# returaj/gan_mpc

Hardware: AMD Instinct MI355X
Metric: trajectories/sec (rollout+backward+critic step) at batch=1024, H=50 (higher is better)
Workload: dtype f32

## Files before the change

### gan_mpc_amd/csrc/gmpc_linearize_sparse.hip

```cpp
#include <cstdio>
#include <type_traits>

#include "gmpc_launch.h"

typedef float f32x4 __attribute__((ext_vector_type(4)));
typedef unsigned v4u __attribute__((ext_vector_type(4)));
typedef unsigned v2u __attribute__((ext_vector_type(2)));

#define GMPC_LIN_PADROWS 24
#define GMPC_SP_H 200
#define GMPC_SP_Z 200
#define GMPC_SP_STR 220
#define GMPC_SP_CAP 216
#define GMPC_SP_WAVE_BYTES (16 * GMPC_SP_STR * 4 + 3 * GMPC_SP_CAP * 4)
#define GMPC_SP_RD 3
#define GMPC_SP_ROW 256

static bool sparse_form(int L, const int* dims, int n, int m) {
  const int Lh = L - 1;
  if (Lh < 2 || n + m > 32 || n < 1) return false;
  for (int l = 1; l <= Lh; ++l)
    if (dims[l] != GMPC_SP_H) return false;
  return true;
}

__global__ void k_pack_sparse(const float* W, float* dst) {
  const int e = blockIdx.x * blockDim.x + threadIdx.x;
  if (e >= GMPC_SP_H * GMPC_SP_H) return;
  const int i = e / GMPC_SP_H, o = e - i * GMPC_SP_H;
  const int t = i >> 4;
  const int slot = i < 192 ? 64 * (t >> 2) + 4 * (i & 15) + (t & 3) : i;
  dst[(size_t)o * GMPC_SP_ROW + slot] = W[e];
}

size_t gmpc_linsparse_floats(int L, const int* dims, int n, int m) {
  if (!sparse_form(L, dims, n, m)) return 0;
  return (size_t)(L - 2) * (GMPC_SP_H + GMPC_LIN_PADROWS) * GMPC_SP_ROW + GMPC_SP_ROW;
}

void gmpc_linsparse_prepare(const MlpDesc& dyn, int n, int m, float* p, LinPad* out, hipStream_t s) {
  for (int l = 0; l < GMPC_MAX_LAYERS; ++l) out->WSP[l] = nullptr;
  if (!sparse_form(dyn.L, dyn.dims, n, m)) return;
  p = reinterpret_cast<float*>((reinterpret_cast<uintptr_t>(p) + 1023) & ~(uintptr_t)1023);
  for (int l = 1; l < dyn.L - 1; ++l) {
    out->WSP[l] = p;
    hipLaunchKernelGGL(k_pack_sparse, dim3((GMPC_SP_H * GMPC_SP_H + 255) / 256), dim3(256), 0, s, dyn.W[l], p);
    p += (size_t)(GMPC_SP_H + GMPC_LIN_PADROWS) * GMPC_SP_ROW;
  }
}

__global__ __launch_bounds__(GMPC_THREADS, 2) void k_linearize_sparse(
    int NSamp, int T, int n, int m, int Lh, LinPad lp, const uint32_t* masks, const int* active, float* AB,
    int samp_mul, int samp_add) {
  extern __shared__ __attribute__((aligned(16))) char smem[];
  const int lane = threadIdx.x & 63, wave = __builtin_amdgcn_readfirstlane(threadIdx.x >> 6);
  const int g = lane >> 4, l16 = lane & 15;
  const int nm = n + m;
  const int nrow = n < 16 ? n : 16;
  char* wbase = smem + wave * GMPC_SP_WAVE_BYTES;
  float* st = reinterpret_cast<float*>(wbase);
  unsigned* lk = reinterpret_cast<unsigned*>(wbase + 16 * GMPC_SP_STR * 4);
  unsigned* lt = lk + GMPC_SP_CAP;
  if (lane < 16 * 8) st[(lane >> 3) * GMPC_SP_STR + GMPC_SP_H + (lane & 7)] = 0.f;
  if (lane + 64 < 16 * 8) st[((lane + 64) >> 3) * GMPC_SP_STR + GMPC_SP_H + (lane & 7)] = 0.f;

  const int lw = l16 * 16, lwt = (192 + (l16 & 7)) * 4;
  const int ls = l16 * GMPC_SP_STR * 4;
  const int tsel = l16 >= 8 ? 1 : 0;
  const unsigned* lkl = lk + g;
  const unsigned* ltl_ = lt + 2 * g + tsel;
  const int lsn = l16 < n ? l16 * 4 : (1 << 28);
  const __amdgpu_buffer_rsrc_t rsl = __builtin_amdgcn_make_buffer_rsrc(
      const_cast<float*>(lp.WLP), 0, (GMPC_SP_H + GMPC_LIN_PADROWS) * n * (int)sizeof(float), 0x00020000);
  const __amdgpu_buffer_rsrc_t rs0 = __builtin_amdgcn_make_buffer_rsrc(
      const_cast<float*>(lp.WTP[0]), 0, (GMPC_SP_H + GMPC_LIN_PADROWS) * 32 * (int)sizeof(float), 0x00020000);

  constexpr int WPB = GMPC_THREADS / 64;
  for (int s = blockIdx.x * WPB + wave; s < NSamp; s += gridDim.x * WPB) {
    const size_t sid = (size_t)s * samp_mul + samp_add;
    if (active != nullptr && active[sid / T] == 0) continue;
    const uint32_t* mrow = masks + sid * Lh * GMPC_MW;

    auto build = [&](int ml) -> int {
      __builtin_amdgcn_wave_barrier();
      int base = 0;
#pragma unroll
      for (int c = 0; c < 4; ++c) {
        const uint32_t lo = __builtin_amdgcn_readfirstlane(mrow[ml * GMPC_MW + 2 * c]);
        uint32_t hi = c < 3 ? __builtin_amdgcn_readfirstlane(mrow[ml * GMPC_MW + 2 * c + 1]) : 0u;
        const uint32_t lo_m = c < 3 ? lo : (lo & 0xFFu);
        const uint32_t word = lane < 32 ? lo_m : hi;
        const int pos = base + (int)__builtin_amdgcn_mbcnt_hi(hi, __builtin_amdgcn_mbcnt_lo(lo_m, 0u));
        const unsigned u = 64 * c + lane;
        if ((word >> (lane & 31)) & 1u) {
          const bool odd = (u & 1u) != 0;
          lk[pos] = u;
          *reinterpret_cast<v2u*>(lt + 2 * pos) = v2u{odd ? GMPC_SP_Z : u, odd ? u : GMPC_SP_Z};
        }
        base += __builtin_popcount(lo_m) + __builtin_popcount(hi);
      }
      if (lane < 16) {
        lk[base + lane] = GMPC_SP_Z;
        *reinterpret_cast<v2u*>(lt + 2 * (base + lane)) = v2u{GMPC_SP_Z, GMPC_SP_Z};
      }
      __builtin_amdgcn_wave_barrier();
      return base;
    };

    auto layer = [&](int l, auto seedc) __attribute__((always_inline)) {
      constexpr bool seed = decltype(seedc)::value;
      const int np = (build(l) + 3) >> 2;
      const __amdgpu_buffer_rsrc_t wrs = __builtin_amdgcn_make_buffer_rsrc(
          const_cast<float*>(lp.WSP[l]), 0, (GMPC_SP_H + GMPC_LIN_PADROWS) * GMPC_SP_ROW * 4, 0x00020000);
      f32x4 acc[13];
      struct Ops { float w[13]; float b; unsigned k, kt; };
      Ops r[GMPC_SP_RD];
      auto tables = [&](Ops& o, int p) {
        o.k = lkl[4 * p];
        o.kt = ltl_[8 * p];
      };
      auto loads = [&](Ops& o) {
        const int k = (int)o.k, kt = (int)o.kt;
        const int vo = (k << 10) + lw, vt = (kt << 10) + lwt;
#pragma unroll
        for (int q = 0; q < 3; ++q) {
          const v4u a = __builtin_amdgcn_raw_buffer_load_b128(wrs, vo + 256 * q, 0, 0);
          o.w[4 * q] = __uint_as_float(a.x); o.w[4 * q + 1] = __uint_as_float(a.y);
          o.w[4 * q + 2] = __uint_as_float(a.z); o.w[4 * q + 3] = __uint_as_float(a.w);
        }
        o.w[12] = __uint_as_float(__builtin_amdgcn_raw_buffer_load_b32(wrs, vt, 0, 0));
        if constexpr (seed) o.b = __uint_as_float(__builtin_amdgcn_raw_buffer_load_b32(rsl, k * n * 4 + lsn, 0, 0));
        else o.b = st[(ls >> 2) + k];
      };
      auto step = [&](int p, Ops& cur, Ops& ahead2) __attribute__((always_inline)) {
        loads(ahead2);
        tables(cur, p + 3);
        __builtin_amdgcn_sched_barrier(0);
#pragma unroll
        for (int t = 0; t < 13; ++t) acc[t] = __builtin_amdgcn_mfma_f32_16x16x4f32(cur.w[t], cur.b, acc[t], 0, 0, 0);
        __builtin_amdgcn_sched_barrier(0);
      };
      if (np == 0) {
#pragma unroll
        for (int t = 0; t < 13; ++t) acc[t] = f32x4{0.f, 0.f, 0.f, 0.f};
      } else {
        tables(r[0], 0); tables(r[1], 1); tables(r[2], 2);
        loads(r[0]); loads(r[1]);
        loads(r[2]);
        tables(r[0], 3);
        __builtin_amdgcn_sched_barrier(0);
#pragma unroll
        for (int t = 0; t < 13; ++t)
          acc[t] = __builtin_amdgcn_mfma_f32_16x16x4f32(r[0].w[t], r[0].b, f32x4{0.f, 0.f, 0.f, 0.f}, 0, 0, 0);
        __builtin_amdgcn_sched_barrier(0);
        int p = 1;
        for (; p + 3 <= np; p += 3) {
          step(p, r[1], r[0]);
          step(p + 1, r[2], r[1]);
          step(p + 2, r[0], r[2]);
        }
        if (p < np) step(p, r[1], r[0]);
        if (p + 1 < np) step(p + 1, r[2], r[1]);
      }
      mfma_fence<false>(acc[0], acc[1], acc[2], acc[3], acc[4], acc[5], acc[6], acc[7], acc[8], acc[9], acc[10],
                        acc[11], acc[12]);
      __builtin_amdgcn_wave_barrier();
      float* srow = st + l16 * GMPC_SP_STR;
#pragma unroll
      for (int t = 0; t < 12; ++t)
        *reinterpret_cast<f32x4*>(srow + 32 * (t >> 1) + 16 * (t & 1) + 4 * g) = acc[t];
      *reinterpret_cast<f32x4*>(srow + (g < 2 ? 192 : 200) + 4 * g) = acc[12];
      __builtin_amdgcn_wave_barrier();
      if (g < 2) {
        const f32x4 x = *reinterpret_cast<const f32x4*>(srow + 192 + 4 * g);
        const f32x4 y = *reinterpret_cast<const f32x4*>(srow + 208 + 4 * g);
        *reinterpret_cast<f32x4*>(srow + 192 + 4 * g) = x + y;
      }
      __builtin_amdgcn_wave_barrier();
    };
    layer(Lh - 1, std::true_type{});
    for (int l = Lh - 2; l >= 1; --l) layer(l, std::false_type{});

    {
      const int np = (build(0) + 3) >> 2;
      f32x4 acc0 = {0.f, 0.f, 0.f, 0.f}, acc1 = {0.f, 0.f, 0.f, 0.f};
      const bool two = nm > 16;
      struct Ops0 { float w0, w1, b; unsigned k; };
      Ops0 r[GMPC_SP_RD];
      auto tables = [&](Ops0& o, int p) { o.k = lkl[4 * p]; };
      auto loads = [&](Ops0& o) {
        const int vo = (int)(o.k << 7) + l16 * 4;
        o.w0 = __uint_as_float(__builtin_amdgcn_raw_buffer_load_b32(rs0, vo, 0, 0));
        o.w1 = __uint_as_float(__builtin_amdgcn_raw_buffer_load_b32(rs0, vo + 64, 0, 0));
        o.b = st[(ls >> 2) + o.k];
      };
      auto step = [&](int p, Ops0& cur, Ops0& ahead2) __attribute__((always_inline)) {
        loads(ahead2);
        tables(cur, p + 3);
        __builtin_amdgcn_sched_barrier(0);
        acc0 = __builtin_amdgcn_mfma_f32_16x16x4f32(cur.w0, cur.b, acc0, 0, 0, 0);
        acc1 = __builtin_amdgcn_mfma_f32_16x16x4f32(cur.w1, cur.b, acc1, 0, 0, 0);
        __builtin_amdgcn_sched_barrier(0);
      };
      tables(r[0], 0); tables(r[1], 1); tables(r[2], 2);
      loads(r[0]); loads(r[1]);
      int p = 0;
      for (; p + 3 <= np; p += 3) {
        step(p, r[0], r[2]);
        step(p + 1, r[1], r[0]);
        step(p + 2, r[2], r[1]);
      }
      if (p < np) step(p, r[0], r[2]);
      if (p + 1 < np) step(p + 1, r[1], r[0]);
      mfma_fence<false>(acc0, acc1);
      if (l16 < nrow) {
        float* dst = AB + ((size_t)s * n + l16) * nm;
#pragma unroll
        for (int j = 0; j < 4; ++j) {
          const int c = 4 * g + j;
          if (c < nm) dst[c] = acc0[j] + (c == l16 ? 1.0f : 0.0f);
          if (two && c + 16 < nm) dst[c + 16] = acc1[j] + (c + 16 == l16 ? 1.0f : 0.0f);
        }
      }
    }
    __builtin_amdgcn_wave_barrier();
  }
}

int gmpc_launch_linearize_sparse(int NSamp, int T, int n, int m, const MlpDesc& dyn, const LinPad& lp,
                                 const uint32_t* masks, const int* active, float* AB, int samp_mul, int samp_add,
                                 hipStream_t s) {
  const int Lh = dyn.L - 1;
  if (!sparse_form(dyn.L, dyn.dims, n, m) || lp.NT != 7 || lp.NTF != 1 || lp.NGF != 1) return -1;
  if (NSamp <= 0) return 0;
  if (n > 16 && gmpc_launch_linearize_regs_rows(NSamp, T, n, m, dyn, lp, masks, active, AB, samp_mul, samp_add, 16,
                                                s) != 0)
    return -1;
  const size_t lds = (size_t)(GMPC_THREADS / 64) * GMPC_SP_WAVE_BYTES;
  int grid = (NSamp + 3) / 4;
  if (grid > 256 * 2) grid = 256 * 2;
  hipLaunchKernelGGL(k_linearize_sparse, dim3(grid), dim3(GMPC_THREADS), lds, s, NSamp, T, n, m, Lh, lp, masks,
                     active, AB, samp_mul, samp_add);
  return 0;
}
```

Measured before the change: 803,800.

## Compact sparse Jacobian linearization to output-active columns with double-buffered index lists

Each hidden layer now builds the next layer's active-index list ahead of time, using double-buffered lists in shared memory. The MFMA accumulation tiles are specialized by template to the number of active output columns (4, 6, 7, 8, 10 or full 12). In the partial cases only the tiles for active output units are computed, using gathered scalar weight loads, and the results are written in compacted order. The next layer then reads its B operand contiguously instead of through the index table. This cuts MFMA and weight-load work when masks are sparse, at the cost of more template instantiations, scalar gathers replacing 128-bit loads, and a hand-placed s_nop hazard wait.

New measurement: 758,000. 0.943x the previous value.

```diff
diff --git a/gan_mpc_amd/csrc/gmpc_linearize_sparse.hip b/gan_mpc_amd/csrc/gmpc_linearize_sparse.hip
--- a/gan_mpc_amd/csrc/gmpc_linearize_sparse.hip
+++ b/gan_mpc_amd/csrc/gmpc_linearize_sparse.hip
@@ -12,7 +12,9 @@
 #define GMPC_SP_Z 200
 #define GMPC_SP_STR 220
 #define GMPC_SP_CAP 216
-#define GMPC_SP_WAVE_BYTES (16 * GMPC_SP_STR * 4 + 3 * GMPC_SP_CAP * 4)
+#define GMPC_SP_LIST (3 * GMPC_SP_CAP)
+#define GMPC_SP_WAVE_BYTES (16 * GMPC_SP_STR * 4 + 2 * GMPC_SP_LIST * 4)
+#define GMPC_SP_FULL_NT 10
 #define GMPC_SP_RD 3
 #define GMPC_SP_ROW 256
 
@@ -59,36 +61,37 @@
   const int nrow = n < 16 ? n : 16;
   char* wbase = smem + wave * GMPC_SP_WAVE_BYTES;
   float* st = reinterpret_cast<float*>(wbase);
-  unsigned* lk = reinterpret_cast<unsigned*>(wbase + 16 * GMPC_SP_STR * 4);
-  unsigned* lt = lk + GMPC_SP_CAP;
-  if (lane < 16 * 8) st[(lane >> 3) * GMPC_SP_STR + GMPC_SP_H + (lane & 7)] = 0.f;
-  if (lane + 64 < 16 * 8) st[((lane + 64) >> 3) * GMPC_SP_STR + GMPC_SP_H + (lane & 7)] = 0.f;
+  unsigned* lists = reinterpret_cast<unsigned*>(wbase + 16 * GMPC_SP_STR * 4);
 
   const int lw = l16 * 16, lwt = (192 + (l16 & 7)) * 4;
-  const int ls = l16 * GMPC_SP_STR * 4;
   const int tsel = l16 >= 8 ? 1 : 0;
-  const unsigned* lkl = lk + g;
-  const unsigned* ltl_ = lt + 2 * g + tsel;
+  float* srow = st + l16 * GMPC_SP_STR;
   const int lsn = l16 < n ? l16 * 4 : (1 << 28);
   const __amdgpu_buffer_rsrc_t rsl = __builtin_amdgcn_make_buffer_rsrc(
       const_cast<float*>(lp.WLP), 0, (GMPC_SP_H + GMPC_LIN_PADROWS) * n * (int)sizeof(float), 0x00020000);
   const __amdgpu_buffer_rsrc_t rs0 = __builtin_amdgcn_make_buffer_rsrc(
       const_cast<float*>(lp.WTP[0]), 0, (GMPC_SP_H + GMPC_LIN_PADROWS) * 32 * (int)sizeof(float), 0x00020000);
 
+  struct List { int buf, cnt, c192; unsigned tail; };
+
   constexpr int WPB = GMPC_THREADS / 64;
   for (int s = blockIdx.x * WPB + wave; s < NSamp; s += gridDim.x * WPB) {
     const size_t sid = (size_t)s * samp_mul + samp_add;
     if (active != nullptr && active[sid / T] == 0) continue;
     const uint32_t* mrow = masks + sid * Lh * GMPC_MW;
 
-    auto build = [&](int ml) -> int {
+    auto build = [&](int ml, int buf) -> List {
+      unsigned* lk = lists + buf * GMPC_SP_LIST;
+      unsigned* lt = lk + GMPC_SP_CAP;
       __builtin_amdgcn_wave_barrier();
       int base = 0;
+      unsigned tail = 0;
 #pragma unroll
       for (int c = 0; c < 4; ++c) {
         const uint32_t lo = __builtin_amdgcn_readfirstlane(mrow[ml * GMPC_MW + 2 * c]);
         uint32_t hi = c < 3 ? __builtin_amdgcn_readfirstlane(mrow[ml * GMPC_MW + 2 * c + 1]) : 0u;
         const uint32_t lo_m = c < 3 ? lo : (lo & 0xFFu);
+        if (c == 3) tail = lo_m;
         const uint32_t word = lane < 32 ? lo_m : hi;
         const int pos = base + (int)__builtin_amdgcn_mbcnt_hi(hi, __builtin_amdgcn_mbcnt_lo(lo_m, 0u));
         const unsigned u = 64 * c + lane;
@@ -104,14 +107,29 @@
         *reinterpret_cast<v2u*>(lt + 2 * (base + lane)) = v2u{GMPC_SP_Z, GMPC_SP_Z};
       }
       __builtin_amdgcn_wave_barrier();
-      return base;
+      return List{buf, base, base - __builtin_popcount(tail), tail};
     };
 
-    auto layer = [&](int l, auto seedc) __attribute__((always_inline)) {
+    auto layer = [&](int l, auto seedc, auto ntc, const List& in, const List& out) __attribute__((always_inline)) {
       constexpr bool seed = decltype(seedc)::value;
-      const int np = (build(l) + 3) >> 2;
+      constexpr int NT = decltype(ntc)::value;
+      constexpr bool full = NT == 12;
+      const int np = (in.cnt + 3) >> 2;
+      const unsigned* lko = lists + out.buf * GMPC_SP_LIST;
+      const unsigned* lkl = lists + in.buf * GMPC_SP_LIST + g;
+      const unsigned* ltl_ = lkl - g + GMPC_SP_CAP + 2 * g + tsel;
+      const float* bp = srow + g;
       const __amdgpu_buffer_rsrc_t wrs = __builtin_amdgcn_make_buffer_rsrc(
           const_cast<float*>(lp.WSP[l]), 0, (GMPC_SP_H + GMPC_LIN_PADROWS) * GMPC_SP_ROW * 4, 0x00020000);
+      int col[NT];
+      if constexpr (!full) {
+#pragma unroll
+        for (int t = 0; t < NT; ++t) {
+          const int pos = 16 * t + l16;
+          const unsigned u = lko[pos];
+          col[t] = pos < out.c192 ? (int)(256 * (u >> 6) + 16 * (u & 15) + 4 * ((u >> 4) & 3)) : GMPC_SP_Z * 4;
+        }
+      }
       f32x4 acc[13];
       struct Ops { float w[13]; float b; unsigned k, kt; };
       Ops r[GMPC_SP_RD];
@@ -119,40 +137,64 @@
         o.k = lkl[4 * p];
         o.kt = ltl_[8 * p];
       };
-      auto loads = [&](Ops& o) {
+      auto loads = [&](Ops& o, int p) {
         const int k = (int)o.k, kt = (int)o.kt;
-        const int vo = (k << 10) + lw, vt = (kt << 10) + lwt;
-#pragma unroll
-        for (int q = 0; q < 3; ++q) {
-          const v4u a = __builtin_amdgcn_raw_buffer_load_b128(wrs, vo + 256 * q, 0, 0);
-          o.w[4 * q] = __uint_as_float(a.x); o.w[4 * q + 1] = __uint_as_float(a.y);
-          o.w[4 * q + 2] = __uint_as_float(a.z); o.w[4 * q + 3] = __uint_as_float(a.w);
-        }
-        o.w[12] = __uint_as_float(__builtin_amdgcn_raw_buffer_load_b32(wrs, vt, 0, 0));
+        if constexpr (full) {
+          const int vo = (k << 10) + lw;
+#pragma unroll
+          for (int q = 0; q < 3; ++q) {
+            const v4u a = __builtin_amdgcn_raw_buffer_load_b128(wrs, vo + 256 * q, 0, 0);
+            o.w[4 * q] = __uint_as_float(a.x); o.w[4 * q + 1] = __uint_as_float(a.y);
+            o.w[4 * q + 2] = __uint_as_float(a.z); o.w[4 * q + 3] = __uint_as_float(a.w);
+          }
+        } else {
+#pragma unroll
+          for (int t = 0; t < NT; ++t)
+            o.w[t] = __uint_as_float(__builtin_amdgcn_raw_buffer_load_b32(wrs, (k << 10) + col[t], 0, 0));
+        }
+        o.w[12] = __uint_as_float(__builtin_amdgcn_raw_buffer_load_b32(wrs, (kt << 10) + lwt, 0, 0));
         if constexpr (seed) o.b = __uint_as_float(__builtin_amdgcn_raw_buffer_load_b32(rsl, k * n * 4 + lsn, 0, 0));
-        else o.b = st[(ls >> 2) + k];
+        else o.b = bp[4 * p];
+      };
+      auto mfmas = [&](const Ops& o, auto first) __attribute__((always_inline)) {
+        __builtin_amdgcn_sched_barrier(0);
+        const f32x4 zero = {0.f, 0.f, 0.f, 0.f};
+#pragma unroll
+        for (int t = 0; t < NT; ++t)
+          acc[t] = __builtin_amdgcn_mfma_f32_16x16x4f32(o.w[t], o.b, decltype(first)::value ? zero : acc[t], 0, 0, 0);
+        acc[12] = __builtin_amdgcn_mfma_f32_16x16x4f32(o.w[12], o.b, decltype(first)::value ? zero : acc[12], 0, 0, 0);
+        __builtin_amdgcn_sched_barrier(0);
       };
       auto step = [&](int p, Ops& cur, Ops& ahead2) __attribute__((always_inline)) {
-        loads(ahead2);
+        loads(ahead2, p + 2);
         tables(cur, p + 3);
-        __builtin_amdgcn_sched_barrier(0);
-#pragma unroll
-        for (int t = 0; t < 13; ++t) acc[t] = __builtin_amdgcn_mfma_f32_16x16x4f32(cur.w[t], cur.b, acc[t], 0, 0, 0);
-        __builtin_amdgcn_sched_barrier(0);
-      };
-      if (np == 0) {
+        mfmas(cur, std::false_type{});
+      };
+      if constexpr (!full) {
+#pragma unroll
+        for (int t = 0; t < 13; ++t) acc[t] = f32x4{0.f, 0.f, 0.f, 0.f};
+        tables(r[0], 0); tables(r[1], 1); tables(r[2], 2);
+        loads(r[0], 0); loads(r[1], 1);
+        int p = 0;
+        if (np >= 3) {
+          do {
+            step(p, r[0], r[2]);
+            step(p + 1, r[1], r[0]);
+            step(p + 2, r[2], r[1]);
+            p += 3;
+          } while (p + 3 <= np);
+        }
+        if (p < np) step(p, r[0], r[2]);
+        if (p + 1 < np) step(p + 1, r[1], r[0]);
+      } else if (np == 0) {
 #pragma unroll
         for (int t = 0; t < 13; ++t) acc[t] = f32x4{0.f, 0.f, 0.f, 0.f};
       } else {
         tables(r[0], 0); tables(r[1], 1); tables(r[2], 2);
-        loads(r[0]); loads(r[1]);
-        loads(r[2]);
+        loads(r[0], 0); loads(r[1], 1);
+        loads(r[2], 2);
         tables(r[0], 3);
-        __builtin_amdgcn_sched_barrier(0);
-#pragma unroll
-        for (int t = 0; t < 13; ++t)
-          acc[t] = __builtin_amdgcn_mfma_f32_16x16x4f32(r[0].w[t], r[0].b, f32x4{0.f, 0.f, 0.f, 0.f}, 0, 0, 0);
-        __builtin_amdgcn_sched_barrier(0);
+        mfmas(r[0], std::true_type{});
         int p = 1;
         for (; p + 3 <= np; p += 3) {
           step(p, r[1], r[0]);
@@ -162,40 +204,82 @@
         if (p < np) step(p, r[1], r[0]);
         if (p + 1 < np) step(p + 1, r[2], r[1]);
       }
-      mfma_fence<false>(acc[0], acc[1], acc[2], acc[3], acc[4], acc[5], acc[6], acc[7], acc[8], acc[9], acc[10],
-                        acc[11], acc[12]);
-      __builtin_amdgcn_wave_barrier();
-      float* srow = st + l16 * GMPC_SP_STR;
-#pragma unroll
-      for (int t = 0; t < 12; ++t)
-        *reinterpret_cast<f32x4*>(srow + 32 * (t >> 1) + 16 * (t & 1) + 4 * g) = acc[t];
-      *reinterpret_cast<f32x4*>(srow + (g < 2 ? 192 : 200) + 4 * g) = acc[12];
-      __builtin_amdgcn_wave_barrier();
-      if (g < 2) {
-        const f32x4 x = *reinterpret_cast<const f32x4*>(srow + 192 + 4 * g);
-        const f32x4 y = *reinterpret_cast<const f32x4*>(srow + 208 + 4 * g);
-        *reinterpret_cast<f32x4*>(srow + 192 + 4 * g) = x + y;
+#pragma unroll
+      for (int t = 0; t < 13; ++t)
+        if (t < NT || t == 12) mfma_tie<false>(acc[t]);
+      asm volatile("s_nop 7\n\ts_nop 7\n\ts_nop 1");
+#pragma unroll
+      for (int t = 0; t < 13; ++t)
+        if (t < NT || t == 12) mfma_tie<false>(acc[t]);
+      __builtin_amdgcn_wave_barrier();
+#pragma unroll
+      for (int t = 0; t < NT; ++t) *reinterpret_cast<f32x4*>(srow + 16 * t + 4 * g) = acc[t];
+      *reinterpret_cast<f32x4*>(srow + 200 + 4 * g) = acc[12];
+      __builtin_amdgcn_wave_barrier();
+      const f32x4 tsum = *reinterpret_cast<const f32x4*>(srow + 200 + 4 * (g & 1)) +
+                         *reinterpret_cast<const f32x4*>(srow + 208 + 4 * (g & 1));
+      __builtin_amdgcn_wave_barrier();
+      if constexpr (!full) {
+        if (g < 3) {
+          *reinterpret_cast<f32x4*>(srow + 16 * NT + 8 * g) = f32x4{0.f, 0.f, 0.f, 0.f};
+          *reinterpret_cast<f32x4*>(srow + 16 * NT + 8 * g + 4) = f32x4{0.f, 0.f, 0.f, 0.f};
+        }
+        __builtin_amdgcn_wave_barrier();
+        if (g < 2) {
+#pragma unroll
+          for (int j = 0; j < 4; ++j) {
+            const unsigned bit = 1u << (4 * g + j);
+            if (out.tail & bit) srow[out.c192 + __builtin_popcount(out.tail & (bit - 1u))] = tsum[j];
+          }
+        }
+      } else {
+        if (g < 2) *reinterpret_cast<f32x4*>(srow + 192 + 4 * g) = tsum;
+        __builtin_amdgcn_wave_barrier();
+        for (int q = g; q < out.cnt + 11; q += 4) {
+          const float v = srow[lko[q]];
+          srow[q] = q < out.cnt ? v : 0.f;
+        }
       }
       __builtin_amdgcn_wave_barrier();
     };
-    layer(Lh - 1, std::true_type{});
-    for (int l = Lh - 2; l >= 1; --l) layer(l, std::false_type{});
-
+    auto hidden = [&](int l, auto seedc, const List& in, const List& out) __attribute__((always_inline)) {
+      const int nt = (out.c192 + 15) >> 4;
+      if (nt <= 4) layer(l, seedc, std::integral_constant<int, 4>{}, in, out);
+      else if (nt <= 6) layer(l, seedc, std::integral_constant<int, 6>{}, in, out);
+      else if (nt == 7) layer(l, seedc, std::integral_constant<int, 7>{}, in, out);
+      else if (nt == 8) layer(l, seedc, std::integral_constant<int, 8>{}, in, out);
+      else if (nt <= GMPC_SP_FULL_NT) layer(l, seedc, std::integral_constant<int, GMPC_SP_FULL_NT>{}, in, out);
+      else layer(l, seedc, std::integral_constant<int, 12>{}, in, out);
+    };
+    List in = build(Lh - 1, 0);
     {
-      const int np = (build(0) + 3) >> 2;
+      const List out = build(Lh - 2, 1);
+      hidden(Lh - 1, std::true_type{}, in, out);
+      in = out;
+    }
+    for (int l = Lh - 2; l >= 1; --l) {
+      const List out = build(l - 1, in.buf ^ 1);
+      hidden(l, std::false_type{}, in, out);
+      in = out;
+    }
+
+    {
+      const int np = (in.cnt + 3) >> 2;
+      const unsigned* lkl = lists + in.buf * GMPC_SP_LIST + g;
+      const float* bp = srow + g;
       f32x4 acc0 = {0.f, 0.f, 0.f, 0.f}, acc1 = {0.f, 0.f, 0.f, 0.f};
       const bool two = nm > 16;
       struct Ops0 { float w0, w1, b; unsigned k; };
       Ops0 r[GMPC_SP_RD];
       auto tables = [&](Ops0& o, int p) { o.k = lkl[4 * p]; };
-      auto loads = [&](Ops0& o) {
+      auto loads = [&](Ops0& o, int p) {
         const int vo = (int)(o.k << 7) + l16 * 4;
         o.w0 = __uint_as_float(__builtin_amdgcn_raw_buffer_load_b32(rs0, vo, 0, 0));
         o.w1 = __uint_as_float(__builtin_amdgcn_raw_buffer_load_b32(rs0, vo + 64, 0, 0));
-        o.b = st[(ls >> 2) + o.k];
+        o.b = bp[4 * p];
       };
       auto step = [&](int p, Ops0& cur, Ops0& ahead2) __attribute__((always_inline)) {
-        loads(ahead2);
+        loads(ahead2, p + 2);
         tables(cur, p + 3);
         __builtin_amdgcn_sched_barrier(0);
         acc0 = __builtin_amdgcn_mfma_f32_16x16x4f32(cur.w0, cur.b, acc0, 0, 0, 0);
@@ -203,7 +287,7 @@
         __builtin_amdgcn_sched_barrier(0);
       };
       tables(r[0], 0); tables(r[1], 1); tables(r[2], 2);
-      loads(r[0]); loads(r[1]);
+      loads(r[0], 0); loads(r[1], 1);
       int p = 0;
       for (; p + 3 <= np; p += 3) {
         step(p, r[0], r[2]);
```
